# caumente/multi_task_breast_cancer

Hardware: AMD Instinct MI355X
Metric: training images/sec (1-ch 256x256, U-Net++ MT) (higher is better)
Workload: dtype bf16; 1 GPU; MTUNetPlusPlus seg+cls deep-supervision step (Dice+Focal, alpha=0.5, Adam eps 1e-4), per-GPU batch 32, 1x256x256, bf16 MFMA operands (3x3 convs, ConvT) and 16-bit stored conv outputs / activations; fp32 accumulation, gradient sums, statistics, losses, parameters and optimizer, random-init weights (BASELINE.json configs[1]); global_batch=32, parallelism=dp1

## Files before the change

multi_task_breast_cancer_amd/csrc/common.h:

```cpp
#pragma once
#include <hip/hip_runtime.h>
#include <stdint.h>
#include <stdlib.h>
#include "../../include/mtbc.h"

#define MTBC_WAVE 64

typedef float f32x4 __attribute__((ext_vector_type(4)));

#define MTBC_CHECK_LAUNCH()                                   \
    do {                                                      \
        hipError_t e__ = hipGetLastError();                   \
        if (e__ != hipSuccess) return MTBC_E_LAUNCH;          \
    } while (0)

#ifdef MTBC_PROBES
#include <stdlib.h>
static inline int mtbc_probe_int(const char* name, int dflt) { const char* v = getenv(name); return v ? atoi(v) : dflt; }
static inline bool mtbc_probe_set(const char* name) { return getenv(name) != nullptr; }
#define MTBC_DBG_BIT(p, bit) ((p).dbg & (bit))
#else
#define mtbc_probe_int(name, dflt) (dflt)
#define mtbc_probe_set(name) (false)
#define MTBC_DBG_BIT(p, bit) (0)
// ... 93 lines not shown
    const bool inb = rx >= 0.f && rx < (float)W && ry >= 0.f && ry < (float)H;
    xs = inb ? (int)rx : 0; ys = inb ? (int)ry : 0;
    if (fh) xs = W - 1 - xs;
    if (fv) ys = H - 1 - ys;
    return inb;
}

__device__ __forceinline__ float block_sum(float v, float* red) {
    const int lane = threadIdx.x & 63, wid = threadIdx.x >> 6, nw = (blockDim.x + 63) >> 6;
    v = wave_sum(v);
    __syncthreads();
    if (lane == 0) red[wid] = v;
    __syncthreads();
    float s = 0.f;
    for (int i = 0; i < nw; ++i) s += red[i];
    return s;
}

enum NormKernel {
    NK_FWD_C8, NK_BWD_C8,
    NK_STATS_FIN, NK_APPLY_FWD, NK_BSTATS_FIN, NK_APPLY_BWD,
    NK_R1_FIN, NK_DPARAM,
    NK_FWD_REG, NK_CHUNK_STATS, NK_CHUNK_APPLY, NK_FWD_STREAM, NK_BWD, NK_BWD_REG
};
struct NormLaunch { int k; int t[6]; int threads; int T, rounds; };
struct NormChoice {
    static constexpr int MAX = 4;
    int n; NormLaunch l[MAX];
    void add(int k, int t0 = 0, int t1 = 0, int t2 = 0, int t3 = 0, int t4 = 0, int t5 = 0) { if (n == MAX) abort(); l[n++] = NormLaunch{k, {t0, t1, t2, t3, t4, t5}, 0, 0, 0}; }
    void add(const NormLaunch& k) { if (n == MAX) abort(); l[n++] = k; }
    NormLaunch& last() { return l[n - 1]; }
};
extern "C" int mtbc_i_instnorm_fwd_c8(const mtbc_instnorm_args* a, hipStream_t st, NormChoice* query);
extern "C" int mtbc_i_instnorm_bwd_c8(const mtbc_instnorm_args* a, float* part, hipStream_t st, NormChoice* query);
extern "C" int mtbc_i_instnorm_bwd_c8_team(const mtbc_instnorm_args* a);
int mtbc_i_maxpool_c8_fwd(const mtbc_maxpool_args* a, hipStream_t st);
int mtbc_i_maxpool_c8_bwd(const mtbc_maxpool_args* a, hipStream_t st);
int mtbc_i_conv1x1_c8_fwd(const mtbc_conv1x1_args* a, hipStream_t st);
size_t mtbc_i_conv1x1_c8_wgrad_workspace(const mtbc_conv1x1_args* a);
int mtbc_i_conv1x1_c8_wgrad(const mtbc_conv1x1_args* a, hipStream_t st);
int mtbc_i_splitk_reduce(const float* partial, float* out, int nsplit, size_t elems, int accumulate, hipStream_t st);
int mtbc_i_splitk_reduce2(const float* partial, float* out, float* out2, int nsplit, size_t elems1, size_t elems2, int accumulate, hipStream_t st);
bool mtbc_i_convT2_fwd_ok(const mtbc_convT_args* a);
int mtbc_i_convT2_fwd(const mtbc_convT_args* a, hipStream_t st);
bool mtbc_i_convT2_fwd_c8_ok(const mtbc_convT_args* a);
int mtbc_i_convT2_fwd_c8(const mtbc_convT_args* a, hipStream_t st);
bool mtbc_i_convT2_fwd_lp_c8_ok(const mtbc_convT_args* a);
int mtbc_i_convT2_fwd_lp_c8(const mtbc_convT_args* a, hipStream_t st);
bool mtbc_i_convT2_dgrad_ok(const mtbc_convT_args* a);
bool mtbc_i_convT2_wgrad_ok(const mtbc_convT_args* a);
void mtbc_i_convT2_wgrad_plan(const mtbc_convT_args* a, int* steps_per_split, int* nsplit);
int mtbc_i_convT2_dgrad(const mtbc_convT_args* a, int compute, hipStream_t st);
int mtbc_i_convT2_wgrad(const mtbc_convT_args* a, int compute, float* partial, float* dbias_part, int steps_per_split, int nsplit, hipStream_t st);
int mtbc_i_channel_sums(const float* x, float* planes_ws, float* out, int N, int C, int HW, int accumulate, hipStream_t st);
```

multi_task_breast_cancer_amd/csrc/convt2.hip:

```cpp
#include "common.h"
#include <utility>

namespace {

typedef __bf16 bf16x8 __attribute__((ext_vector_type(8)));
typedef _Float16 f16x8 __attribute__((ext_vector_type(8)));

template <int LP> struct Frag;
template <> struct Frag<0> {
    float v[8];
    __device__ __forceinline__ void set(const float* f) {
#pragma unroll
        for (int i = 0; i < 8; ++i) v[i] = f[i];
    }
    static __device__ __forceinline__ f32x4 mma(const Frag& a, const Frag& b, f32x4 c) {
#pragma unroll
        for (int i = 0; i < 8; ++i) c = __builtin_amdgcn_mfma_f32_16x16x4f32(a.v[i], b.v[i], c, 0, 0, 0);
        return c;
    }
};
template <> struct Frag<1> {
    bf16x8 v;
    __device__ __forceinline__ void set(const float* f) {
#pragma unroll
// ... 734 lines not shown
            constexpr int slot = decltype(SL)::value;
            const unsigned short* q = dyn16 + (size_t)(8 * s) * 4 * HW;
#pragma unroll
            for (int c = 0; c < 2; ++c) {
                rh[slot][2 * c] = *reinterpret_cast<const uint2*>(q + (size_t)c * 4 * HW);
                rh[slot][2 * c + 1] = *reinterpret_cast<const uint2*>(q + (size_t)c * 4 * HW + oW);
            }
        };
        auto compute = [&](int s, auto SL) {
            constexpr int cur = decltype(SL)::value;
            Frag<LP> fe, fo;
            frag_from_words<LP>(fe, rh[cur][0].x, rh[cur][1].x, rh[cur][2].x, rh[cur][3].x);
            frag_from_words<LP>(fo, rh[cur][0].y, rh[cur][1].y, rh[cur][2].y, rh[cur][3].y);
#pragma unroll
            for (int m = 0; m < MT; ++m) {
                Frag<LP> fa;
                fa.v = __builtin_bit_cast(decltype(fa.v), *reinterpret_cast<const ct_u32x4*>(arow + (size_t)(m * 16) * wrow + 32 * s));
                acc[m][0] = Frag<LP>::mma(fa, fe, acc[m][0]);
                acc[m][1] = Frag<LP>::mma(fa, fo, acc[m][1]);
            }
        };
        sfor<D - 1>([&](auto U) { load(min((int)U.value, last), U); });
        int s = 0;
        for (; s + D <= nsteps; s += D)
            sfor<D>([&](auto U) {
                constexpr int u = decltype(U)::value;
                load(min(s + u + D - 1, last), SC<(u + D - 1) % D>{});
                __builtin_amdgcn_sched_barrier(0);
                compute(s + u, U);
                __builtin_amdgcn_sched_barrier(0);
            });
        sfor<D - 1>([&](auto U) { if (s + U.value < nsteps) compute(s + U.value, U); });
        float* dxn = p.dx + (size_t)n * p.dxbs + g * 32 + 2 * j;
        float2 old[MT][4];
        if (p.acc_dx) {
#pragma unroll
            for (int m = 0; m < MT; ++m)
#pragma unroll
                for (int r = 0; r < 4; ++r) old[m][r] = *reinterpret_cast<const float2*>(dxn + (size_t)min(mb * 48 + m * 16 + kg * 4 + r, p.Cin - 1) * HW);
        }
#pragma unroll
        for (int m = 0; m < MT; ++m)
#pragma unroll
            for (int r = 0; r < 4; ++r) {
                const int ci = mb * 48 + m * 16 + kg * 4 + r;
                if (ci >= p.Cin) continue;
                float2 v = make_float2(acc[m][0][r], acc[m][1][r]);
                if (p.acc_dx) { v.x += old[m][r].x; v.y += old[m][r].y; }
                *reinterpret_cast<float2*>(dxn + (size_t)ci * HW) = v;
            }
    }
}

bool al16(const void* q) { return (reinterpret_cast<uintptr_t>(q) & 15) == 0; }

void fill(const mtbc_convT_args* a, Ct2P* p) {
    p->N = a->N; p->H = a->H; p->W = a->W; p->Cin = a->Cin; p->Cout = a->Cout;
    p->x = a->x; p->xbs = a->x_batch_stride; p->w = a->w; p->dy = a->dy; p->dybs = a->dy_batch_stride;
    p->dx = a->dx; p->dxbs = a->dx_batch_stride; p->acc_dx = a->accumulate_dx; p->partial = nullptr; p->dbias_part = nullptr;
    p->mblocks = cdiv(a->Cin, 48); p->ctiles = cdiv(a->Cout, 8); p->steps_per_split = 1; p->nsplit = 1; p->ntasks = 0; p->xcd_tasks = 0;
}

}

bool mtbc_i_convT2_dgrad_ok(const mtbc_convT_args* a) {
    const int HW = a->H * a->W;
    if (a->dy_type16 && (a->dy_type16 != a->compute || a->dy_batch_stride % 8 != 0)) return false;
    return a->k == 2 && HW % 32 == 0 && a->W % 2 == 0 && a->Cout % 2 == 0 && al16(a->dy) && al16(a->w) && al16(a->dx) &&
           a->dy_batch_stride % 4 == 0 && a->dx_batch_stride % 2 == 0;
}
bool mtbc_i_convT2_wgrad_ok(const mtbc_convT_args* a) {
    const int HW = a->H * a->W;
    if (a->dy_type16 && (a->dy_type16 != a->compute || a->dy_batch_stride % 8 != 0)) return false;
    if (a->x_type16 && (a->x_type16 != a->compute || !a->dy_type16 || a->x_batch_stride % 8 != 0)) return false;
    return a->k == 2 && HW % 32 == 0 && a->W % 8 == 0 && al16(a->dy) && al16(a->x) && a->dy_batch_stride % 4 == 0 &&
           a->x_batch_stride % 4 == 0;
}
void mtbc_i_convT2_wgrad_plan(const mtbc_convT_args* a, int* steps_per_split, int* nsplit) {
    const long long total_steps = (long long)a->N * (a->H * a->W / 32);
    const long long per_split_tasks = (long long)cdiv(a->Cin, 48) * cdiv(a->Cout, 8);
    static const int tasks_env = mtbc_probe_int("MTBC_CT_WG_TASKS", 0);
    long long want = cdiv64(tasks_env > 0 ? tasks_env : (a->x_type16 ? 1536 : 4096), per_split_tasks);
    if (want < 1) want = 1;
    long long sps = cdiv64(total_steps, want);
    if (sps < 8) sps = 8;
    if (sps > total_steps) sps = total_steps;
    *steps_per_split = (int)sps;
    *nsplit = (int)cdiv64(total_steps, sps);
}

bool mtbc_i_convT2_fwd_ok(const mtbc_convT_args* a) {
    const int HW = a->H * a->W;
    return a->k == 2 && HW % 32 == 0 && a->W % 2 == 0 && a->Cin % 4 == 0 && a->Cin <= 4 * FKI && 4 * a->Cout <= 16 * FMT &&
           al16(a->x) && al16(a->y) && al16(a->w) && a->x_batch_stride % 2 == 0 && a->y_batch_stride % 4 == 0;
}
int mtbc_i_convT2_fwd(const mtbc_convT_args* a, hipStream_t st) {
    Ct2P p; fill(a, &p);
    const int wstride = (4 * a->Cout + 31) / 32 * 32 + 16;
    const size_t lds = (size_t)a->Cin * wstride * sizeof(float);
    const long long groups = (long long)a->N * (a->H * a->W / 32);
    int blocks = (int)(groups < 4 * 512 ? cdiv64(groups, 4) : 512);
    const int ki = cdiv(a->Cin, 4);
#define MTBC_CT2F(KI_)                                                                                                     \
    do {                                                                                                                   \
        MTBC_ENSURE_DYN_LDS((&convT2_fwd_lds_kernel<KI_>), 64 * 1024);                                                     \
        hipLaunchKernelGGL(convT2_fwd_lds_kernel<KI_>, dim3(blocks), dim3(256), lds, st, p, a->bias, a->y,                 \
                           (long long)a->y_batch_stride, wstride);                                                         \
    } while (0)
    if (ki <= 8) MTBC_CT2F(8); else if (ki <= 12) MTBC_CT2F(12); else MTBC_CT2F(16);
#undef MTBC_CT2F
    MTBC_CHECK_LAUNCH();
    return MTBC_OK;
}

bool mtbc_i_convT2_fwd_c8_ok(const mtbc_convT_args* a) {
    const int HW = a->H * a->W, cp = (a->Cout + 15) / 16 * 16;
    return a->k == 2 && HW % 32 == 0 && a->Cin % 4 == 0 && a->Cin <= 4 * FKI && 4 * cp <= 16 * FMT && a->Cout % 8 == 0 &&
           (a->y_type == 1 || a->y_type == 2) && al16(a->y) && a->y_batch_stride % 8 == 0;
}
int mtbc_i_convT2_fwd_c8(const mtbc_convT_args* a, hipStream_t st) {
    Ct2P p; fill(a, &p);
    const int cp = (a->Cout + 15) / 16 * 16;
    const int wstride = (4 * cp + 31) / 32 * 32 + 16;
    const size_t lds = ((size_t)a->Cin * wstride + cp) * sizeof(float);
    const long long groups = (long long)a->N * (a->H * a->W / 32);
    int blocks = (int)(groups < 4 * 512 ? cdiv64(groups, 4) : 512);
    const int ki = cdiv(a->Cin, 4);
    unsigned short* y8 = reinterpret_cast<unsigned short*>(a->y);
#define MTBC_CT2F8(KI_, F16_)                                                                                              \
    do {                                                                                                                   \
// ... 67 lines not shown
#undef MTBC_CT2DG
        MTBC_CHECK_LAUNCH();
        return MTBC_OK;
    }
    static const int depth_env = mtbc_probe_int("MTBC_CT_DEPTH", 0);
    const bool deep = depth_env ? depth_env >= 4 : a->Cout >= 96;
    if (a->dy_type16) {
        if (compute == 1) { if (deep) hipLaunchKernelGGL((convT2_dgrad_kernel<1, true, 4>), dim3(blocks), dim3(256), 0, st, p); else hipLaunchKernelGGL((convT2_dgrad_kernel<1, true>), dim3(blocks), dim3(256), 0, st, p); }
        else { if (deep) hipLaunchKernelGGL((convT2_dgrad_kernel<2, true, 4>), dim3(blocks), dim3(256), 0, st, p); else hipLaunchKernelGGL((convT2_dgrad_kernel<2, true>), dim3(blocks), dim3(256), 0, st, p); }
    } else if (compute == 1) hipLaunchKernelGGL(convT2_dgrad_kernel<1>, dim3(blocks), dim3(256), 0, st, p);
    else if (compute == 2) hipLaunchKernelGGL(convT2_dgrad_kernel<2>, dim3(blocks), dim3(256), 0, st, p);
    else hipLaunchKernelGGL(convT2_dgrad_kernel<0>, dim3(blocks), dim3(256), 0, st, p);
    MTBC_CHECK_LAUNCH();
    return MTBC_OK;
}

int mtbc_i_convT2_wgrad(const mtbc_convT_args* a, int compute, float* partial, float* dbias_part, int steps_per_split, int nsplit, hipStream_t st) {
    Ct2P p; fill(a, &p);
    p.partial = partial; p.dbias_part = dbias_part; p.steps_per_split = steps_per_split; p.nsplit = nsplit;
    p.ntasks = (long long)p.mblocks * p.ctiles * nsplit;
    const unsigned blocks = (unsigned)cdiv64(p.ntasks, 4);
    if (a->x_type16) {
        if (!a->dy_type16 || a->x_type16 != compute) return MTBC_E_UNSUPPORTED;
        static const int ct_env = mtbc_probe_int("MTBC_CT_WG_CT", 0);
        const int ctn = ct_env ? ct_env : (p.ctiles % 2 == 0 ? 2 : 1);
        static const int xcd_env = mtbc_probe_int("MTBC_CT_WG_XCD", 1);
        const long long pst = (long long)p.mblocks * cdiv(p.ctiles, ctn);
        const long long per_xcd = (long long)cdiv(nsplit, 8) * pst;
        unsigned xblocks = 0;
        if (xcd_env && nsplit >= 8 && per_xcd < (1ll << 30)) { p.xcd_tasks = (int)per_xcd; xblocks = 8u * (unsigned)cdiv64(per_xcd, 4); }
        if (ctn == 2) {
            p.ntasks = (long long)p.mblocks * ((p.ctiles + 1) / 2) * nsplit;
            const unsigned b2 = xblocks ? xblocks : (unsigned)cdiv64(p.ntasks, 4);
            static const int depth_env = mtbc_probe_int("MTBC_CT_DEPTH", 2);
            if (depth_env == 2) {
                if (compute == 1) hipLaunchKernelGGL((convT2_wgrad16_kernel<1, 2, 2>), dim3(b2), dim3(256), 0, st, p);
                else hipLaunchKernelGGL((convT2_wgrad16_kernel<2, 2, 2>), dim3(b2), dim3(256), 0, st, p);
            } else if (compute == 1) hipLaunchKernelGGL((convT2_wgrad16_kernel<1, 2, 4>), dim3(b2), dim3(256), 0, st, p);
            else hipLaunchKernelGGL((convT2_wgrad16_kernel<2, 2, 4>), dim3(b2), dim3(256), 0, st, p);
        } else {
            const unsigned b1 = xblocks ? xblocks : blocks;
            if (compute == 1) hipLaunchKernelGGL((convT2_wgrad16_kernel<1, 1, 4>), dim3(b1), dim3(256), 0, st, p);
            else hipLaunchKernelGGL((convT2_wgrad16_kernel<2, 1, 4>), dim3(b1), dim3(256), 0, st, p);
        }
    } else if (a->dy_type16) {
        if (compute == 1) hipLaunchKernelGGL((convT2_wgrad_kernel<1, true>), dim3(blocks), dim3(256), 0, st, p);
        else hipLaunchKernelGGL((convT2_wgrad_kernel<2, true>), dim3(blocks), dim3(256), 0, st, p);
    } else if (compute == 1) hipLaunchKernelGGL(convT2_wgrad_kernel<1>, dim3(blocks), dim3(256), 0, st, p);
    else if (compute == 2) hipLaunchKernelGGL(convT2_wgrad_kernel<2>, dim3(blocks), dim3(256), 0, st, p);
    else hipLaunchKernelGGL(convT2_wgrad_kernel<0>, dim3(blocks), dim3(256), 0, st, p);
    MTBC_CHECK_LAUNCH();
    return MTBC_OK;
}
```

multi_task_breast_cancer_amd/csrc/pool_up.hip:

```cpp
#include "common.h"
#include <cstdlib>

namespace {

constexpr int GRS = 81;

template <bool A_KCONTIG, bool B_KCONTIG, class AL, class BL, class CS>
__device__ __forceinline__ void gemm_block_64x64(int m0, int c0, int kbeg, int kend, AL al, BL bl, CS cs) {
    constexpr int BK = 32;
    __shared__ float As[BK * GRS];
    __shared__ float Bs[BK * GRS];
    const int tid = threadIdx.x, lane = tid & 63, wv = tid >> 6;
    const int j = lane & 15, kk = lane >> 4;
    const int mrow = 32 * (wv >> 1), ccol = 32 * (wv & 1);
    f32x4 acc[2][2];
#pragma unroll
    for (int a = 0; a < 2; ++a)
#pragma unroll
        for (int b = 0; b < 2; ++b) acc[a][b] = (f32x4){0.f, 0.f, 0.f, 0.f};

    float ra[8], rb[8];
    auto fetch = [&](int k0) {
#pragma unroll
        for (int i = 0; i < 8; ++i) {
// ... 410 lines not shown
    if ((a->H * a->W) & 3) return MTBC_E_UNSUPPORTED;
    p->N = a->N; p->HW = a->H * a->W; p->Cin = a->Cin; p->Cout = a->Cout; p->x = a->x; p->xbs = a->x_batch_stride;
    p->w = a->w; p->bias = a->bias; p->y = a->y; p->dy = a->dy; p->dx = a->dx; p->dxbs = a->dx_batch_stride;
    p->acc_dx = a->accumulate_dx; p->partial = nullptr;
    return MTBC_OK;
}
int mtbc_conv1x1_fwd(const mtbc_conv1x1_args* a, void* stream) {
    C1P p; int rc = fill_c1(a, &p); if (rc) return rc;
    if (!p.x || !p.w || !p.y) return MTBC_E_BADARG;
    if (a->x_layout == MTBC_LAYOUT_C8) return mtbc_i_conv1x1_c8_fwd(a, (hipStream_t)stream);
    if (a->x_layout != MTBC_LAYOUT_PLANAR) return MTBC_E_BADARG;
    if (!al16(p.x) || !al16(p.y) || (p.xbs & 3)) return MTBC_E_UNSUPPORTED;
    dim3 grid(cdiv(p.HW / 4, 256), cdiv(a->Cout, 8), a->N);
    hipLaunchKernelGGL(conv1x1_fwd_kernel, grid, dim3(256), 0, (hipStream_t)stream, p);
    MTBC_CHECK_LAUNCH();
    return MTBC_OK;
}
int mtbc_conv1x1_dgrad(const mtbc_conv1x1_args* a, void* stream) {
    C1P p; int rc = fill_c1(a, &p); if (rc) return rc;
    if (!p.dy || !p.w || !p.dx) return MTBC_E_BADARG;
    if (!al16(p.dy) || !al16(p.dx) || (p.dxbs & 3)) return MTBC_E_UNSUPPORTED;
    dim3 grid(cdiv(p.HW / 4, 256), 1, a->N);
    hipLaunchKernelGGL(conv1x1_dgrad_kernel, grid, dim3(256), 0, (hipStream_t)stream, p);
    MTBC_CHECK_LAUNCH();
    return MTBC_OK;
}
size_t mtbc_conv1x1_wgrad_workspace(const mtbc_conv1x1_args* a) {
    if (!a) return 0;
    if (a->x_layout == MTBC_LAYOUT_C8) return mtbc_i_conv1x1_c8_wgrad_workspace(a);
    return ((size_t)a->N * a->Cout * a->Cin + (size_t)a->N * a->Cout) * sizeof(float);
}
int mtbc_conv1x1_wgrad(const mtbc_conv1x1_args* a, void* stream) {
    C1P p; int rc = fill_c1(a, &p); if (rc) return rc;
    if (!p.x || !p.dy || !a->dw) return MTBC_E_BADARG;
    if (a->x_layout == MTBC_LAYOUT_C8) return mtbc_i_conv1x1_c8_wgrad(a, (hipStream_t)stream);
    if (a->x_layout != MTBC_LAYOUT_PLANAR) return MTBC_E_BADARG;
    if (!al16(p.x) || !al16(p.dy) || (p.xbs & 3)) return MTBC_E_UNSUPPORTED;
    if (!a->workspace || a->workspace_bytes < mtbc_conv1x1_wgrad_workspace(a)) return MTBC_E_WORKSPACE;
    p.partial = reinterpret_cast<float*>(a->workspace);
    hipStream_t st = (hipStream_t)stream;
    hipLaunchKernelGGL(conv1x1_wgrad_kernel, dim3(a->Cin, a->N), dim3(256), 0, st, p);
    MTBC_CHECK_LAUNCH();
    const size_t wel = (size_t)a->Cout * a->Cin;
    rc = mtbc_i_splitk_reduce(p.partial, a->dw, a->N, wel, a->accumulate_dw, st); if (rc) return rc;
    if (a->dbias) {
        rc = mtbc_i_channel_sums(p.dy, p.partial + (size_t)a->N * wel, a->dbias, a->N, a->Cout, p.HW, a->accumulate_dw, st);
        if (rc) return rc;
    }
    return MTBC_OK;
}

}

namespace {
__global__ void head_combine_kernel(const mtbc_head_fuse_args a) {
    const int kk = a.k * a.k;
    const int idx = blockIdx.x * blockDim.x + threadIdx.x;
    const int total = a.Cin * a.R * kk;
    if (idx < total) {
        const int ab = idx % kk, r = (idx / kk) % a.R, ci = idx / (kk * a.R);
        float s = 0.f;
        for (int co = 0; co < a.Cmid; ++co) s = fmaf(a.wT[((size_t)ci * a.Cmid + co) * kk + ab], a.w1[(size_t)r * a.Cmid + co], s);
        a.Wc[idx] = s;
    }
    if (idx < a.R) {
        float s = a.b1 ? a.b1[idx] : 0.f;
        if (a.bT) for (int co = 0; co < a.Cmid; ++co) s = fmaf(a.bT[co], a.w1[(size_t)idx * a.Cmid + co], s);
        a.bc[idx] = s;
    }
}
__global__ void head_expand_dwT_kernel(const mtbc_head_fuse_args a) {
    const int kk = a.k * a.k;
    const int idx = blockIdx.x * blockDim.x + threadIdx.x;
    const int total = a.Cin * a.Cmid * kk;
    if (idx >= total) return;
    const int ab = idx % kk, co = (idx / kk) % a.Cmid, ci = idx / (kk * a.Cmid);
    float s = 0.f;
    for (int r = 0; r < a.R; ++r) s = fmaf(a.G[((size_t)ci * a.R + r) * kk + ab], a.w1[(size_t)r * a.Cmid + co], s);
    a.dwT[idx] = a.acc_wT ? a.dwT[idx] + s : s;
}
__global__ void head_expand_small_kernel(const mtbc_head_fuse_args a) {
    __shared__ float red[32];
    const int r = blockIdx.x / a.Cmid, co = blockIdx.x % a.Cmid, kk = a.k * a.k;
    float s = 0.f;
    for (int i = threadIdx.x; i < a.Cin * kk; i += blockDim.x) {
        const int ci = i / kk, ab = i % kk;
        s = fmaf(a.G[((size_t)ci * a.R + r) * kk + ab], a.wT[((size_t)ci * a.Cmid + co) * kk + ab], s);
    }
    s = block_sum(s, red);
    if (threadIdx.x != 0) return;
    if (a.bT) s = fmaf(a.gb[r], a.bT[co], s);
    a.dw1[(size_t)r * a.Cmid + co] = a.acc_w1 ? a.dw1[(size_t)r * a.Cmid + co] + s : s;
    if (r == 0 && a.dbT) {
        float t = 0.f;
        for (int q = 0; q < a.R; ++q) t = fmaf(a.gb[q], a.w1[(size_t)q * a.Cmid + co], t);
        a.dbT[co] = a.acc_bT ? a.dbT[co] + t : t;
    }
    if (co == 0 && a.db1) a.db1[r] = a.acc_b1 ? a.db1[r] + a.gb[r] : a.gb[r];
}
}

extern "C" int mtbc_convT_head_combine(const mtbc_head_fuse_args* a, void* stream) {
    if (!a || !a->wT || !a->w1 || !a->Wc || !a->bc) return MTBC_E_BADARG;
    if (a->Cin <= 0 || a->Cmid <= 0 || a->R <= 0 || a->k <= 0) return MTBC_E_BADSHAPE;
    const int total = a->Cin * a->R * a->k * a->k;
    hipLaunchKernelGGL(head_combine_kernel, dim3(cdiv(total > a->R ? total : a->R, 128)), dim3(128), 0, (hipStream_t)stream, *a);
// ... 14 lines not shown
```

multi_task_breast_cancer_amd/csrc/program.hip:

```cpp
#include "common.h"

extern "C" {

int mtbc_version(void) { return MTBC_VERSION; }
const char* mtbc_arch(void) { return "gfx950"; }

const char* mtbc_strerror(int code) {
    switch (code) {
        case MTBC_OK: return "ok";
        case MTBC_E_BADSHAPE: return "bad shape";
        case MTBC_E_BADARG: return "bad argument (null or misaligned pointer)";
        case MTBC_E_WORKSPACE: return "workspace missing or too small";
        case MTBC_E_LAUNCH: return "kernel launch failed";
        case MTBC_E_UNSUPPORTED: return "unsupported configuration";
        default: return "unknown error";
    }
}

static inline bool is_pack(int32_t k) { return k == MTBC_OP_CONV3_PACK_FWD || k == MTBC_OP_CONV3_PACK_DGRAD || k == MTBC_OP_CONV3_PACK_LP; }

int mtbc_event_create(void** event) {
    if (!event) return MTBC_E_BADARG;
    hipEvent_t e;
    if (hipEventCreateWithFlags(&e, hipEventDisableTiming) != hipSuccess) return MTBC_E_LAUNCH;
// ... 22 lines not shown
            continue;
        }
        if (o->kind == MTBC_OP_EVENT_RECORD || o->kind == MTBC_OP_EVENT_WAIT) {
            hipError_t e = hipErrorInvalidValue;
            if (o->u.sync.event)
                e = o->kind == MTBC_OP_EVENT_RECORD ? hipEventRecord((hipEvent_t)o->u.sync.event, (hipStream_t)stream)
                                                    : hipStreamWaitEvent((hipStream_t)stream, (hipEvent_t)o->u.sync.event, 0);
            if (e != hipSuccess) { if (failed_index) *failed_index = i; return o->u.sync.event ? MTBC_E_LAUNCH : MTBC_E_BADARG; }
            continue;
        }
        if (is_pack(o->kind)) {
            mtbc_pack_desc d[128];
            int32_t n = 0;
            while (n < 128 && i + n < first + count && is_pack(ops[i + n].kind)) {
                const mtbc_op* q = &ops[i + n];
                d[n].w = q->u.pack.w; d[n].packed = q->u.pack.packed; d[n].Cin = q->u.pack.Cin; d[n].Cout = q->u.pack.Cout;
                d[n].compute = q->u.pack.compute;
                d[n].kind = q->kind == MTBC_OP_CONV3_PACK_FWD ? 0 : q->kind == MTBC_OP_CONV3_PACK_DGRAD ? 1 : (q->u.pack.dgrad ? 3 : 2);
                ++n;
            }
            if (n > 1) {
                rc = mtbc_conv3x3_pack_many(d, n, stream);
                if (rc != MTBC_OK) { if (failed_index) *failed_index = i; return rc; }
                i += n - 1;
                continue;
            }
        }
        if (o->kind == MTBC_OP_CONV3_WVIEW) {
            mtbc_wview_desc d[128];
            int32_t n = 0;
            while (n < 128 && i + n < first + count && ops[i + n].kind == MTBC_OP_CONV3_WVIEW) {
                const mtbc_op* q = &ops[i + n];
                d[n].w = q->u.wview.w; d[n].dst = q->u.wview.dst; d[n].Cout = q->u.wview.Cout; d[n].Cin = q->u.wview.Cin;
                d[n].ci_off = q->u.wview.ci_off; d[n].ci_cnt = q->u.wview.ci_cnt; d[n].mode = q->u.wview.mode;
                d[n].k_off = q->u.wview.k_off; d[n].K = q->u.wview.K;
                ++n;
            }
            if (n > 1) {
                rc = mtbc_conv3x3_weight_view_many(d, n, stream);
                if (rc != MTBC_OK) { if (failed_index) *failed_index = i; return rc; }
                i += n - 1;
                continue;
            }
        }
        if (o->kind == MTBC_OP_IN_DPARAM) {
            mtbc_dparam_desc d[64];
            int32_t n = 0;
            while (n < 64 && i + n < first + count && ops[i + n].kind == MTBC_OP_IN_DPARAM) { d[n] = ops[i + n].u.dparam; ++n; }
            rc = mtbc_instnorm_dparam_many(d, n, stream);
            if (rc != MTBC_OK) { if (failed_index) *failed_index = i; return rc; }
            i += n - 1;
            continue;
        }
        switch (o->kind) {
            case MTBC_OP_CONV3_FWD: rc = mtbc_conv3x3_fwd(&o->u.conv3, stream); break;
            case MTBC_OP_CONV3_DGRAD: rc = mtbc_conv3x3_dgrad(&o->u.conv3, stream); break;
            case MTBC_OP_CONV3_WGRAD: rc = mtbc_conv3x3_wgrad(&o->u.conv3, stream); break;
            case MTBC_OP_CONV3_PACK_FWD: rc = mtbc_conv3x3_pack_fwd(o->u.pack.w, o->u.pack.packed, o->u.pack.Cin, o->u.pack.Cout, stream); break;
            case MTBC_OP_CONV3_PACK_DGRAD: rc = mtbc_conv3x3_pack_dgrad(o->u.pack.w, o->u.pack.packed, o->u.pack.Cin, o->u.pack.Cout, stream); break;
            case MTBC_OP_HEAD_COMBINE: rc = mtbc_convT_head_combine(&o->u.head, stream); break;
            case MTBC_OP_HEAD_EXPAND: rc = mtbc_convT_head_expand(&o->u.head, stream); break;
            case MTBC_OP_CONV3_WVIEW: rc = mtbc_conv3x3_weight_view(o->u.wview.w, o->u.wview.dst, o->u.wview.Cout, o->u.wview.Cin, o->u.wview.ci_off, o->u.wview.ci_cnt, o->u.wview.mode, o->u.wview.k_off, o->u.wview.K, stream); break;
            case MTBC_OP_C8_PACK16: rc = mtbc_c8_pack16(o->u.c8pack.src, o->u.c8pack.src_batch_stride, o->u.c8pack.dst, o->u.c8pack.N, o->u.c8pack.C, o->u.c8pack.HW, stream); break;
            case MTBC_OP_C8_PACK: rc = mtbc_c8_pack(o->u.c8pack.src, o->u.c8pack.src_batch_stride, o->u.c8pack.dst, o->u.c8pack.N, o->u.c8pack.C, o->u.c8pack.HW, o->u.c8pack.compute, stream); break;
            case MTBC_OP_CONV3_PACK_LP: rc = mtbc_conv3x3_pack_lp(o->u.pack.w, o->u.pack.packed, o->u.pack.Cin, o->u.pack.Cout, o->u.pack.dgrad, o->u.pack.compute, stream); break;
            case MTBC_OP_IN_FWD: rc = mtbc_instnorm_lrelu_fwd(&o->u.inorm, stream); break;
            case MTBC_OP_IN_BWD: rc = mtbc_instnorm_lrelu_bwd(&o->u.inorm, stream); break;
            case MTBC_OP_POOL_FWD: rc = mtbc_maxpool2_fwd(&o->u.pool, stream); break;
            case MTBC_OP_POOL_BWD: rc = mtbc_maxpool2_bwd(&o->u.pool, stream); break;
            case MTBC_OP_CONVT_FWD: rc = mtbc_convT_fwd(&o->u.convT, stream); break;
            case MTBC_OP_CONVT_DGRAD: rc = mtbc_convT_dgrad(&o->u.convT, stream); break;
            case MTBC_OP_CONVT_WGRAD: rc = mtbc_convT_wgrad(&o->u.convT, stream); break;
            case MTBC_OP_CONV1_FWD: rc = mtbc_conv1x1_fwd(&o->u.conv1, stream); break;
            case MTBC_OP_CONV1_DGRAD: rc = mtbc_conv1x1_dgrad(&o->u.conv1, stream); break;
            case MTBC_OP_CONV1_WGRAD: rc = mtbc_conv1x1_wgrad(&o->u.conv1, stream); break;
            case MTBC_OP_GAP_FWD: rc = mtbc_gap_fwd(&o->u.gap, stream); break;
            case MTBC_OP_GAP_BWD: rc = mtbc_gap_bwd(&o->u.gap, stream); break;
            case MTBC_OP_LINEAR_FWD: rc = mtbc_linear_fwd(&o->u.linear, stream); break;
            case MTBC_OP_LINEAR_BWD: rc = mtbc_linear_bwd(&o->u.linear, stream); break;
            case MTBC_OP_DICE_FWD: rc = mtbc_dice_fwd(&o->u.dice, stream); break;
            case MTBC_OP_DICE_BWD: rc = mtbc_dice_bwd(&o->u.dice, stream); break;
            case MTBC_OP_FOCAL: rc = mtbc_focal_fwd_bwd(&o->u.focal, stream); break;
            case MTBC_OP_LOSS_MIX: rc = mtbc_loss_mix(o->u.mix.seg, o->u.mix.cls, o->u.mix.alpha, o->u.mix.out4, stream); break;
            case MTBC_OP_OPTIM: rc = mtbc_optim_step(&o->u.optim, stream); break;
            case MTBC_OP_MEMSET:
                rc = hipMemsetAsync(o->u.memset0.ptr, 0, o->u.memset0.bytes, (hipStream_t)stream) == hipSuccess ? MTBC_OK : MTBC_E_LAUNCH;
                break;
            case MTBC_OP_DICE_COUNTS: rc = mtbc_dice_counts(o->u.counts.logits, o->u.counts.target, o->u.counts.n, o->u.counts.out3, stream); break;
            default: rc = MTBC_E_BADARG;
        }
        if (rc != MTBC_OK) {
            if (failed_index) *failed_index = i;
            return rc;
        }
    }
    return MTBC_OK;
}

}
```

multi_task_breast_cancer_amd/switches.py:

```python
from __future__ import annotations

import os
from typing import Dict, List

PLAN_SWITCHES: Dict[str, tuple] = {
    "MTBC_NO_COOP": ("0", "InstanceNorm by one-plane workgroups (fp32 conv outputs) + pack instead of the channel-group / cooperative kernels: "
                          "the fallback when their teams cannot be co-resident (the cooperative error message names it)",
                     "tests/test_model_gpu.py::test_16bit_mfma_modes_match_their_emulation[...-no_coop-40]"),
    "MTBC_NO_GATHER": ("0", "every 3x3 conv back-propagates into all its inputs (fan-in by read-modify-write) instead of one gathered launch per dense-skip tensor",
                       "tests/test_model_gpu.py::test_16bit_mfma_modes_match_their_emulation[...-no_gather]"),
    "MTBC_NO_Z16": ("0", "16-bit modes keep the conv outputs z as fp32 planes (InstanceNorm reads 4 bytes per element in both directions): the storage arm of the quality sweeps",
                    "tests/test_model_gpu.py::test_16bit_mfma_modes_match_their_emulation[...-no_z16]"),
    "MTBC_Z_BF16": ("0", "bf16 mode stores the conv outputs as bf16 instead of fp16 (same bytes, 8 instead of 11 significant bits)",
                    "tests/test_model_gpu.py::test_16bit_mfma_modes_match_their_emulation[...-z_bf16]"),
    "MTBC_DA16": ("0", "the gradient a conv-cell activation gets from its 3x3 consumers is written by ONE gathered launch as a 16-bit channel-blocked tensor (fp32 sum in the MFMA "
                       "accumulators, one RNE) instead of fp32 planar fan-in: -0.36 ms per step.  Default in round 3 on the easy task's evidence (-0.010 +- 0.025 pt); OFF again since "
                       "round 4: on the task that can fail it ends at the same Dice (-0.012 +- 0.042 pt against fp32, 10 paired seeds) but reaches the plateau LATER -- mid-run "
                       "-5.6 +- 2.9 pt against fp32 where the fp32-gradient plan is at -0.5 +- 1.4 and tracks the fp32 runs seed by seed (profiles/r04_quality_hard.md)",
                  "tests/test_model_gpu.py::test_16bit_mfma_modes_match_their_emulation[...-da16]"),
    "MTBC_NOFUSE_HEADS": ("0", "MTnnUNet deep-supervision heads as ConvT + 1x1 (the reference's two layers) instead of one combined ConvT",
                          "tests/test_model_gpu.py::test_mtnnunet_two_layer_heads_match_the_fused_heads_and_the_oracle"),
    "MTBC_GRAPH": ("0", "trainer.FusedTrainStep (single process) captures each compiled step -- weight images, forward, losses, backward, Adam -- into ONE hipGraph at its third call "
                        "and replays it from then on: the host issues a step in 0.1 ms instead of 8.4 (profiles/r04_graph_replay.txt); the GPU time is the same, the results are the same bits "
                        "(the optimizer's per-step scalars travel through device memory, mtbc_optim_args.dynamic)",
                   "tests/test_model_gpu.py::test_graph_replayed_steps_are_the_eager_steps"),
    "MTBC_DYN_SCALE": ("0", "trainer.FusedTrainStep(loss_scale=None) trains with the device-side dynamic loss scale (loss_scale.DynamicLossScale(): start 2^16, found-inf check "
                            "over the flat gradients, skip + halve on overflow, double after 2000 clean steps) instead of the static scale baked into the loss ops: three more "
                            "launches per step; without an overflow the same bits as the static 2^16 of fp16 mode",
                       "tests/test_loss_scale_gpu.py::test_dynamic_steps_without_overflow_are_the_static_steps"),
    "MTBC_NO_STEM_MC": ("0", "a first conv with intensity channels (data.augmentation: Cin 2 .. 5) takes the launches it took before the multi-channel stem kernels: "
                             "conv3x3_direct_kernel, an fp32 conv output under the one-plane InstanceNorm, the small-Cin (Cin = 5: the direct) weight gradient from fp32 dz -- "
                             "the A arm of tools/stem_cost.py",
                        "tests/test_stem_multichannel_gpu.py::test_whole_model_against_the_emulation[...-no_stem_mc]"),
    "MTBC_COOP_RESERVE_CUS": ("64", "CUs kept out of the cooperative InstanceNorm grids under data parallel",
                              "tests/test_coop_safety_gpu.py::test_cooperative_step_beside_a_cu_hogging_kernel"),
}
REMOVED = ("MTBC_NO_C8", "MTBC_NO_CT_LP", "MTBC_COOP_MIN_FWD", "MTBC_COOP_MIN_BWD", "MTBC_NO_P16", "MTBC_FANIN", "MTBC_NO_C8_SMALL_OPS", "MTBC_NO_X16",
           "MTBC_NO_G16", "MTBC_NO_EPI_STATS", "MTBC_EPI_BSTATS", "MTBC_NO_R1", "MTBC_NO_POOLFOLD", "MTBC_SPLIT_FANIN", "MTBC_NO_STEM16",
           "MTBC_NO_DEFER_DPARAM", "MTBC_DPARAM_BATCH", "MTBC_NO_POOLFWD_FOLD", "MTBC_BWD_OVERLAP", "MTBC_BWD_OVERLAP_MAX_HW",
           "MTBC_NO_DA16")
RESULT_ALTERING = ("MTBC_DBG", "MTBC_NOACC", "MTBC_LOWP", "MTBC_LP_MT", "MTBC_RING", "MTBC_NODMA", "MTBC_C8_BLOCKS_PER_CU",
                   "MTBC_WGRAD_LP1", "MTBC_CT_WG_TASKS", "MTBC_IN_BWD_STREAM", "MTBC_CONVT_GENERIC", "MTBC_C8_NW", "MTBC_C8_RING",
                   "MTBC_CT_DEPTH", "MTBC_CT_WG_CT", "MTBC_CT_WG_XCD", "MTBC_CT_DGRAD_DIRECT", "MTBC_WGRAD_C8W", "MTBC_C8W_BPC", "MTBC_C8W_DEPTH", "MTBC_C8W_HACK",
                   "MTBC_WGRAD_PACK24", "MTBC_WGRAD_C8I", "MTBC_WG_NS8", "MTBC_WG_TS", "MTBC_C8_TS", "MTBC_RING_TS", "MTBC_INB_TS")


def get(name: str) -> str:
    return os.environ.get(name, PLAN_SWITCHES[name][0])


def flag(name: str) -> bool:
    v = get(name)
    return v not in ("", "0")


def active() -> Dict[str, str]:
    return {k: v for k, v in sorted(os.environ.items()) if k.startswith("MTBC_")}


def removed() -> List[str]:
    return [k for k in REMOVED if k in os.environ]


def refuse_removed() -> None:
    bad = removed()
    if bad:
        raise RuntimeError(f"removed plan switch(es) set: {bad} -- these arms no longer exist (switches.py REMOVED; the 16-bit gathered gradients are the opt-in MTBC_DA16=1 since round 4, "
                           "MTBC_NO_DA16 is gone); unset them")


def result_altering() -> List[str]:
    bad = [k for k in RESULT_ALTERING if k in os.environ]
    if "MTBC_LIB" in os.environ:
        bad.append("MTBC_LIB")
    return bad
```

Measured before the change: 2856 images/sec.

## Fuse transposed-conv weight-gradient and data-gradient into one kernel sharing dy loads

Result: faster. 2885 images/sec (median of 6 runs) (+1.0%).

```diff
diff --git a/multi_task_breast_cancer_amd/csrc/common.h b/multi_task_breast_cancer_amd/csrc/common.h
--- a/multi_task_breast_cancer_amd/csrc/common.h
+++ b/multi_task_breast_cancer_amd/csrc/common.h
@@ -169,4 +169,7 @@
 void mtbc_i_convT2_wgrad_plan(const mtbc_convT_args* a, int* steps_per_split, int* nsplit);
 int mtbc_i_convT2_dgrad(const mtbc_convT_args* a, int compute, hipStream_t st);
 int mtbc_i_convT2_wgrad(const mtbc_convT_args* a, int compute, float* partial, float* dbias_part, int steps_per_split, int nsplit, hipStream_t st);
+bool mtbc_i_convT2_bwd_fused_ok(const mtbc_convT_args* wg, const mtbc_convT_args* dg);
+int mtbc_i_convT2_bwd_fused(const mtbc_convT_args* wg, const mtbc_convT_args* dg, float* partial, float* dbias_part, int steps_per_split, int nsplit, hipStream_t st);
+int mtbc_i_convT_bwd_pair(const mtbc_convT_args* wg, const mtbc_convT_args* dg, void* stream, bool* fused);
 int mtbc_i_channel_sums(const float* x, float* planes_ws, float* out, int N, int C, int HW, int accumulate, hipStream_t st);
diff --git a/multi_task_breast_cancer_amd/csrc/convt2.hip b/multi_task_breast_cancer_amd/csrc/convt2.hip
--- a/multi_task_breast_cancer_amd/csrc/convt2.hip
+++ b/multi_task_breast_cancer_amd/csrc/convt2.hip
@@ -810,6 +810,222 @@
     }
 }
 
+constexpr int FDYROW = 80;
+template <int LP, int CT, int NW, bool ACC>
+__global__ __launch_bounds__(64 * NW) void convT2_bwd_fused_kernel(const Ct2P p, const int wrow) {
+    static_assert(LP != 0, "16-bit operands");
+    static_assert(NW == 3 || NW == 6, "3 input-channel tiles x 1 or 2 pixel parities");
+    constexpr int D = 2, NT = 64 * NW, NE = NW == 3 ? 2 : 1;
+    extern __shared__ __attribute__((aligned(16))) unsigned short Lf[];
+    const int tid = threadIdx.x, lane = tid & 63, wv = __builtin_amdgcn_readfirstlane(tid >> 6);
+    const int j = lane & 15, kg = lane >> 4;
+    const int HW = p.H * p.W, oW = 2 * p.W, M4 = 4 * p.Cout;
+    const int steps_per_img = HW / 32;
+    const int kb = (int)(blockIdx.x >> 3);
+    const int split = 8 * (kb / p.mblocks) + (int)(blockIdx.x & 7), mb = kb % p.mblocks;
+    if (split >= p.nsplit) return;
+    unsigned short* Wd = Lf;
+    unsigned short* Dy = Lf + 48 * wrow;
+    const int slot_elems = 2 * p.Cout * FDYROW;
+    const int ppr = M4 / 8, npieces = 48 * ppr;
+    for (int base = tid; base < npieces; base += NT * 4) {
+        float4 v[4][2];
+#pragma unroll
+        for (int u = 0; u < 4; ++u) {
+            const int idx = min(base + NT * u, npieces - 1), r = idx / ppr, q = idx - r * ppr;
+            const float* src = p.w + (size_t)min(mb * 48 + r, p.Cin - 1) * M4 + 8 * q;
+            v[u][0] = ld4(src); v[u][1] = ld4(src + 4);
+        }
+#pragma unroll
+        for (int u = 0; u < 4; ++u) {
+            const int idx = base + NT * u;
+            if (idx >= npieces) continue;
+            const int r = idx / ppr, q = idx - r * ppr;
+            ct_u32x4 o = {cvt_pk16<LP == 2>(v[u][0].x, v[u][0].y), cvt_pk16<LP == 2>(v[u][0].z, v[u][0].w),
+                          cvt_pk16<LP == 2>(v[u][1].x, v[u][1].y), cvt_pk16<LP == 2>(v[u][1].z, v[u][1].w)};
+            if (mb * 48 + r >= p.Cin) o = (ct_u32x4){0u, 0u, 0u, 0u};
+            *reinterpret_cast<ct_u32x4*>(Wd + (size_t)r * wrow + 8 * q) = o;
+        }
+    }
+    __syncthreads();
+
+    const int total_steps = p.N * steps_per_img;
+    const int g0 = split * p.steps_per_split, g1 = min(total_steps, g0 + p.steps_per_split);
+    bool rok[MT];
+    const unsigned short* xrow[MT];
+#pragma unroll
+    for (int m = 0; m < MT; ++m) {
+        const int ci = mb * 48 + m * 16 + j;
+        rok[m] = ci < p.Cin;
+        xrow[m] = reinterpret_cast<const unsigned short*>(p.x) + (size_t)(rok[m] ? ci : 0) * HW + 8 * kg;
+    }
+    int co[CT];
+    const unsigned short* dcol[CT];
+#pragma unroll
+    for (int c = 0; c < CT; ++c) {
+        co[c] = (wv * CT + c) * 8 + (j >> 1);
+        dcol[c] = reinterpret_cast<const unsigned short*>(p.dy) + (size_t)co[c] * 4 * HW + (size_t)(j & 1) * oW;
+    }
+    f32x4 acc[CT][MT][2];
+#pragma unroll
+    for (int c = 0; c < CT; ++c)
+#pragma unroll
+        for (int m = 0; m < MT; ++m) { acc[c][m][0] = (f32x4){0.f, 0.f, 0.f, 0.f}; acc[c][m][1] = (f32x4){0.f, 0.f, 0.f, 0.f}; }
+    const bool want_bias = p.dbias_part != nullptr && mb == 0;
+    float bsum[CT];
+#pragma unroll
+    for (int c = 0; c < CT; ++c) bsum[c] = 0.f;
+    const int dm = NW == 3 ? wv : wv % 3, de = NW == 3 ? 0 : wv / 3;
+    const unsigned short* arow = Wd + (size_t)(dm * 16 + j) * wrow + 8 * kg;
+    unsigned short* dyw = Dy + (size_t)(wv * CT * 16 + j) * FDYROW + 16 * kg;
+    const unsigned short* dyr = Dy + (size_t)(4 * kg) * FDYROW + 4 * j;
+    const int nsteps = p.Cout / 8;
+
+    ct_u32x4 rx[D][MT], rh[D][CT][2];
+    float old[4][NE];
+    auto load = [&](int g, auto SL) {
+        constexpr int slot = decltype(SL)::value;
+        const int n = g / steps_per_img, st = g % steps_per_img;
+        const int pix = st * 32 + 8 * kg;
+        const int i = pix / p.W, jx = pix % p.W;
+#pragma unroll
+        for (int m = 0; m < MT; ++m) rx[slot][m] = *reinterpret_cast<const ct_u32x4*>(xrow[m] + (size_t)n * p.xbs + st * 32);
+#pragma unroll
+        for (int c = 0; c < CT; ++c) {
+            const unsigned short* q = dcol[c] + (size_t)n * p.dybs + (size_t)(2 * i) * oW + 2 * jx;
+            rh[slot][c][0] = *reinterpret_cast<const ct_u32x4*>(q); rh[slot][c][1] = *reinterpret_cast<const ct_u32x4*>(q + 8);
+        }
+    };
+    auto dx_of = [&](int g) {
+        const int n = g / steps_per_img, st = g % steps_per_img;
+        return p.dx + (size_t)n * p.dxbs + st * 32 + 2 * j + de;
+    };
+    auto load_old = [&](int g) {
+        if constexpr (ACC) {
+            const float* dxn = dx_of(g);
+#pragma unroll
+            for (int r = 0; r < 4; ++r) {
+                const float* q = dxn + (size_t)min(mb * 48 + dm * 16 + kg * 4 + r, p.Cin - 1) * HW;
+                if constexpr (NE == 2) { const float2 o = *reinterpret_cast<const float2*>(q); old[r][0] = o.x; old[r][1] = o.y; }
+                else old[r][0] = *q;
+            }
+        }
+    };
+    auto compute = [&](int t, auto SL) {
+        constexpr int cur = decltype(SL)::value;
+        Frag<LP> fa[MT];
+#pragma unroll
+        for (int m = 0; m < MT; ++m) {
+            const ct_u32x4 w = rx[cur][m];
+            frag_from_words<LP>(fa[m], rok[m] ? w[0] : 0u, rok[m] ? w[1] : 0u, rok[m] ? w[2] : 0u, rok[m] ? w[3] : 0u);
+        }
+        unsigned short* sw = dyw + (size_t)(t & 1) * slot_elems;
+#pragma unroll
+        for (int c = 0; c < CT; ++c) {
+            *reinterpret_cast<ct_u32x4*>(sw + (size_t)(c * 16) * FDYROW) = rh[cur][c][0];
+            *reinterpret_cast<ct_u32x4*>(sw + (size_t)(c * 16) * FDYROW + 8) = rh[cur][c][1];
+            unsigned d[8], w0[4], w1[4];
+#pragma unroll
+            for (int k = 0; k < 4; ++k) { d[k] = rh[cur][c][0][k]; d[4 + k] = rh[cur][c][1][k]; }
+#pragma unroll
+            for (int m = 0; m < 4; ++m) {
+                w0[m] = (d[2 * m] & 0xffffu) | (d[2 * m + 1] << 16);
+                w1[m] = (d[2 * m] >> 16) | (d[2 * m + 1] & 0xffff0000u);
+            }
+            if (want_bias) {
+#pragma unroll
+                for (int k = 0; k < 8; ++k) bsum[c] += sum2_16<LP>(d[k]);
+            }
+            Frag<LP> f0, f1;
+            frag_from_words<LP>(f0, w0[0], w0[1], w0[2], w0[3]);
+            frag_from_words<LP>(f1, w1[0], w1[1], w1[2], w1[3]);
+#pragma unroll
+            for (int m = 0; m < MT; ++m) {
+                acc[c][m][0] = Frag<LP>::mma(fa[m], f0, acc[c][m][0]);
+                acc[c][m][1] = Frag<LP>::mma(fa[m], f1, acc[c][m][1]);
+            }
+        }
+    };
+    auto dgrad = [&](int g, int t) {
+        asm volatile("s_waitcnt lgkmcnt(0)\n\ts_barrier" ::: "memory");
+        const unsigned short* sr = dyr + (size_t)(t & 1) * slot_elems;
+        f32x4 da[NE];
+#pragma unroll
+        for (int e = 0; e < NE; ++e) da[e] = (f32x4){0.f, 0.f, 0.f, 0.f};
+        for (int s = 0; s < nsteps; ++s) {
+            uint2 h[4];
+#pragma unroll
+            for (int r = 0; r < 4; ++r) h[r] = *reinterpret_cast<const uint2*>(sr + (size_t)(16 * s + r) * FDYROW);
+            Frag<LP> fa;
+            fa.v = __builtin_bit_cast(decltype(fa.v), *reinterpret_cast<const ct_u32x4*>(arow + 32 * s));
+            if constexpr (NE == 2) {
+                Frag<LP> fe, fo;
+                frag_from_words<LP>(fe, h[0].x, h[1].x, h[2].x, h[3].x);
+                frag_from_words<LP>(fo, h[0].y, h[1].y, h[2].y, h[3].y);
+                da[0] = Frag<LP>::mma(fa, fe, da[0]);
+                da[1] = Frag<LP>::mma(fa, fo, da[1]);
+            } else {
+                Frag<LP> fb;
+                frag_from_words<LP>(fb, de ? h[0].y : h[0].x, de ? h[1].y : h[1].x, de ? h[2].y : h[2].x, de ? h[3].y : h[3].x);
+                da[0] = Frag<LP>::mma(fa, fb, da[0]);
+            }
+        }
+        float* dxn = dx_of(g);
+#pragma unroll
+        for (int r = 0; r < 4; ++r) {
+            const int ci = mb * 48 + dm * 16 + kg * 4 + r;
+            if (ci >= p.Cin) continue;
+            float* q = dxn + (size_t)ci * HW;
+            if constexpr (NE == 2) {
+                float2 v = make_float2(da[0][r], da[1][r]);
+                if constexpr (ACC) { v.x += old[r][0]; v.y += old[r][1]; }
+                *reinterpret_cast<float2*>(q) = v;
+            } else {
+                float v = da[0][r];
+                if constexpr (ACC) v += old[r][0];
+                *q = v;
+            }
+        }
+    };
+    {
+        const int last = g1 - 1;
+        sfor<D - 1>([&](auto U) { load(min(g0 + (int)U.value, last), U); });
+        int g = g0;
+        for (; g + D <= g1; g += D)
+            sfor<D>([&](auto U) {
+                constexpr int u = decltype(U)::value;
+                load_old(g + u);
+                load(min(g + u + D - 1, last), SC<(u + D - 1) % D>{});
+                __builtin_amdgcn_sched_barrier(0);
+                compute(g + u - g0, U);
+                dgrad(g + u, g + u - g0);
+                __builtin_amdgcn_sched_barrier(0);
+            });
+        sfor<D - 1>([&](auto U) {
+            if (g + U.value < g1) { load_old(g + U.value); compute(g + U.value - g0, U); dgrad(g + U.value, g + U.value - g0); }
+        });
+    }
+    float* part = p.partial + (size_t)split * p.Cin * p.Cout * 4;
+#pragma unroll
+    for (int c = 0; c < CT; ++c) {
+        if (want_bias) {
+            float b = bsum[c];
+            b += __shfl_xor(b, 16);
+            b += __shfl_xor(b, 32);
+            b += __shfl_xor(b, 1);
+            if (kg == 0 && (j & 1) == 0) p.dbias_part[(size_t)split * p.Cout + co[c]] = b;
+        }
+#pragma unroll
+        for (int m = 0; m < MT; ++m)
+#pragma unroll
+            for (int r = 0; r < 4; ++r) {
+                const int ci = mb * 48 + m * 16 + kg * 4 + r;
+                if (ci >= p.Cin) continue;
+                *reinterpret_cast<float2*>(part + ((size_t)ci * p.Cout + co[c]) * 4 + 2 * (j & 1)) = make_float2(acc[c][m][0][r], acc[c][m][1][r]);
+            }
+    }
+}
+
 bool al16(const void* q) { return (reinterpret_cast<uintptr_t>(q) & 15) == 0; }
 
 void fill(const mtbc_convT_args* a, Ct2P* p) {
@@ -834,6 +1050,26 @@
     return a->k == 2 && HW % 32 == 0 && a->W % 8 == 0 && al16(a->dy) && al16(a->x) && a->dy_batch_stride % 4 == 0 &&
            a->x_batch_stride % 4 == 0;
 }
+constexpr int FUSED_MIN_BLOCKS = 256;
+static int fused_ct(const mtbc_convT_args* a) { return (a->Cout / 8) % 2 == 0 ? 2 : 1; }
+static size_t fused_lds(const mtbc_convT_args* a) { return (size_t)48 * (4 * a->Cout + 16) * 2 + (size_t)2 * 2 * a->Cout * FDYROW * 2; }
+bool mtbc_i_convT2_bwd_fused_ok(const mtbc_convT_args* wg, const mtbc_convT_args* dg) {
+    if (wg->N != dg->N || wg->H != dg->H || wg->W != dg->W || wg->Cin != dg->Cin || wg->Cout != dg->Cout || wg->k != dg->k ||
+        wg->compute != dg->compute || wg->dy != dg->dy || wg->dy_batch_stride != dg->dy_batch_stride || wg->dy_type16 != dg->dy_type16 ||
+        wg->w != dg->w) return false;
+    if (wg->compute != 1 && wg->compute != 2) return false;
+    if (wg->dy_type16 != wg->compute || wg->x_type16 != wg->compute) return false;
+    if (!mtbc_i_convT2_wgrad_ok(wg) || !mtbc_i_convT2_dgrad_ok(dg)) return false;
+    if (wg->Cout % 8 != 0) return false;
+    const int nw = wg->Cout / 8 / fused_ct(wg);
+    if (nw != 3 && nw != 6) return false;
+    if (fused_lds(wg) > 104 * 1024) return false;
+    static const bool all = mtbc_probe_set("MTBC_CT_FUSE_ALL");
+    int sps, ns; mtbc_i_convT2_wgrad_plan(wg, &sps, &ns);
+    if (!all && (long long)ns * cdiv(wg->Cin, 48) < FUSED_MIN_BLOCKS && sps > 8) return false;
+    return true;
+}
+
 void mtbc_i_convT2_wgrad_plan(const mtbc_convT_args* a, int* steps_per_split, int* nsplit) {
     const long long total_steps = (long long)a->N * (a->H * a->W / 32);
     const long long per_split_tasks = (long long)cdiv(a->Cin, 48) * cdiv(a->Cout, 8);
@@ -1007,3 +1243,32 @@
     MTBC_CHECK_LAUNCH();
     return MTBC_OK;
 }
+
+int mtbc_i_convT2_bwd_fused(const mtbc_convT_args* wg, const mtbc_convT_args* dg, float* partial, float* dbias_part, int steps_per_split, int nsplit, hipStream_t st) {
+    if (!mtbc_i_convT2_bwd_fused_ok(wg, dg)) return MTBC_E_UNSUPPORTED;
+    Ct2P p; fill(wg, &p);
+    p.dx = dg->dx; p.dxbs = dg->dx_batch_stride; p.acc_dx = dg->accumulate_dx;
+    p.partial = partial; p.dbias_part = dbias_part; p.steps_per_split = steps_per_split; p.nsplit = nsplit;
+    const int ctn = fused_ct(wg), nw = p.ctiles / ctn, compute = wg->compute;
+    const int wrow = 4 * wg->Cout + 16;
+    const size_t lds = fused_lds(wg);
+    const long long nblocks = 8ll * cdiv(nsplit, 8) * p.mblocks;
+    if (nblocks >= (1ll << 31)) return MTBC_E_UNSUPPORTED;
+    const dim3 grid((unsigned)nblocks);
+    const bool acc = dg->accumulate_dx != 0;
+#define MTBC_CT2BF(LP_, CT_, NW_, ACC_)                                                                                  \
+    do {                                                                                                                 \
+        MTBC_ENSURE_DYN_LDS((&convT2_bwd_fused_kernel<LP_, CT_, NW_, ACC_>), 104 * 1024);                                \
+        hipLaunchKernelGGL((convT2_bwd_fused_kernel<LP_, CT_, NW_, ACC_>), grid, dim3(64 * NW_), lds, st, p, wrow);      \
+    } while (0)
+#define MTBC_CT2BF_SHAPE(LP_, ACC_)                                                                                      \
+    do {                                                                                                                 \
+        if (ctn == 1) MTBC_CT2BF(LP_, 1, 3, ACC_); else if (nw == 3) MTBC_CT2BF(LP_, 2, 3, ACC_); else MTBC_CT2BF(LP_, 2, 6, ACC_); \
+    } while (0)
+    if (compute == 1) { if (acc) MTBC_CT2BF_SHAPE(1, true); else MTBC_CT2BF_SHAPE(1, false); }
+    else { if (acc) MTBC_CT2BF_SHAPE(2, true); else MTBC_CT2BF_SHAPE(2, false); }
+#undef MTBC_CT2BF_SHAPE
+#undef MTBC_CT2BF
+    MTBC_CHECK_LAUNCH();
+    return MTBC_OK;
+}
diff --git a/multi_task_breast_cancer_amd/csrc/pool_up.hip b/multi_task_breast_cancer_amd/csrc/pool_up.hip
--- a/multi_task_breast_cancer_amd/csrc/pool_up.hip
+++ b/multi_task_breast_cancer_amd/csrc/pool_up.hip
@@ -486,6 +486,26 @@
 
 }
 
+int mtbc_i_convT_bwd_pair(const mtbc_convT_args* wg, const mtbc_convT_args* dg, void* stream, bool* fused) {
+    *fused = false;
+    CtP p;
+    if (fill_ct(wg, &p) != MTBC_OK || fill_ct(dg, &p) != MTBC_OK) return MTBC_OK;
+    if (!wg->x || !wg->dy || !wg->dw || !dg->dy || !dg->w || !dg->dx) return MTBC_OK;
+    static const bool generic = mtbc_probe_set("MTBC_CONVT_GENERIC");
+    static const bool unfused = mtbc_probe_set("MTBC_CT_UNFUSED");
+    if (generic || unfused || !mtbc_i_convT2_bwd_fused_ok(wg, dg)) return MTBC_OK;
+    if (!wg->workspace || wg->workspace_bytes < mtbc_convT_wgrad_workspace(wg)) return MTBC_OK;
+    fill_ct(wg, &p);
+    hipStream_t st = (hipStream_t)stream;
+    int sps, nsplit; mtbc_i_convT2_wgrad_plan(wg, &sps, &nsplit);
+    float* partial = reinterpret_cast<float*>(wg->workspace);
+    float* bpart = wg->dbias ? partial + (size_t)nsplit * wg->Cin * p.M : nullptr;
+    *fused = true;
+    int rc = mtbc_i_convT2_bwd_fused(wg, dg, partial, bpart, sps, nsplit, st); if (rc) return rc;
+    if (bpart) { rc = mtbc_i_splitk_reduce(bpart, wg->dbias, nsplit, (size_t)wg->Cout, wg->accumulate_dw, st); if (rc) return rc; }
+    return mtbc_i_splitk_reduce(partial, wg->dw, nsplit, (size_t)wg->Cin * p.M, wg->accumulate_dw, st);
+}
+
 namespace {
 __global__ void head_combine_kernel(const mtbc_head_fuse_args a) {
     const int kk = a.k * a.k;
diff --git a/multi_task_breast_cancer_amd/csrc/program.hip b/multi_task_breast_cancer_amd/csrc/program.hip
--- a/multi_task_breast_cancer_amd/csrc/program.hip
+++ b/multi_task_breast_cancer_amd/csrc/program.hip
@@ -98,6 +98,12 @@
             i += n - 1;
             continue;
         }
+        if (o->kind == MTBC_OP_CONVT_WGRAD && i + 1 < first + count && ops[i + 1].kind == MTBC_OP_CONVT_DGRAD) {
+            bool fused = false;
+            rc = mtbc_i_convT_bwd_pair(&o->u.convT, &ops[i + 1].u.convT, stream, &fused);
+            if (rc != MTBC_OK) { if (failed_index) *failed_index = i; return rc; }
+            if (fused) { ++i; continue; }
+        }
         switch (o->kind) {
             case MTBC_OP_CONV3_FWD: rc = mtbc_conv3x3_fwd(&o->u.conv3, stream); break;
             case MTBC_OP_CONV3_DGRAD: rc = mtbc_conv3x3_dgrad(&o->u.conv3, stream); break;
diff --git a/multi_task_breast_cancer_amd/switches.py b/multi_task_breast_cancer_amd/switches.py
--- a/multi_task_breast_cancer_amd/switches.py
+++ b/multi_task_breast_cancer_amd/switches.py
@@ -42,7 +42,8 @@
 RESULT_ALTERING = ("MTBC_DBG", "MTBC_NOACC", "MTBC_LOWP", "MTBC_LP_MT", "MTBC_RING", "MTBC_NODMA", "MTBC_C8_BLOCKS_PER_CU",
                    "MTBC_WGRAD_LP1", "MTBC_CT_WG_TASKS", "MTBC_IN_BWD_STREAM", "MTBC_CONVT_GENERIC", "MTBC_C8_NW", "MTBC_C8_RING",
                    "MTBC_CT_DEPTH", "MTBC_CT_WG_CT", "MTBC_CT_WG_XCD", "MTBC_CT_DGRAD_DIRECT", "MTBC_WGRAD_C8W", "MTBC_C8W_BPC", "MTBC_C8W_DEPTH", "MTBC_C8W_HACK",
-                   "MTBC_WGRAD_PACK24", "MTBC_WGRAD_C8I", "MTBC_WG_NS8", "MTBC_WG_TS", "MTBC_C8_TS", "MTBC_RING_TS", "MTBC_INB_TS")
+                   "MTBC_WGRAD_PACK24", "MTBC_WGRAD_C8I", "MTBC_WG_NS8", "MTBC_WG_TS", "MTBC_C8_TS", "MTBC_RING_TS", "MTBC_INB_TS",
+                   "MTBC_CT_UNFUSED", "MTBC_CT_FUSE_ALL")
 
 
 def get(name: str) -> str:
```
